# Gorilla-Lab-SCUT/GeoA3

Hardware: AMD Instinct MI355X
Metric: attack-iterations/sec (B=250, N=1024) (higher is better)
Workload: dtype f32; 1 GPU; configs[1]: PointNet 1024-pt, 250 instances sharded over 1 GPU(s) (250 on rank 0), full GeoA3 (CE + CD 1.0 + HD 0.1 + curvature 1.0 k=16), untargeted; instances_per_gpu=250, global_batch=250, npoint=1024, knn=16, classes=40, wide_mode=f16x2, presteps=150, parallelism=instance-sharded x1

## Files before the change

### geoa3_amd/csrc/pointnet_wide16.hip

```cpp
#include "pointnet_kernels.h"
#include "profile.h"

namespace {

constexpr int W16_THREADS = 256;
constexpr int W16_OCC = 2;
constexpr int W16_PTS = 128;
constexpr int W16_ROWS = W16_PTS + 2;
constexpr int W16_ROWB = 288;
constexpr int W16_PIECEB = W16_ROWS * W16_ROWB;
constexpr int W16_LDS = 2 * W16_PIECEB;

__global__ __launch_bounds__(W16_THREADS, W16_OCC) void wide16_kernel(WideArgs a, int slots_per_xcd) {
  constexpr int TAPS = 3;
  constexpr int GROUPS = 4;
  constexpr int KS = TAPS * 4;
  constexpr int PF = 2;
  extern __shared__ __attribute__((aligned(16))) unsigned char smem_raw[];
  __shared__ float s_max[4];
  __shared__ unsigned long long s_keys[4][GROUPS][32];
  const int tid = threadIdx.x, lane = tid & 63, wave = tid >> 6, p16 = lane & 15, q4 = lane >> 4, l31 = lane & 31,
            kh = lane >> 5;
  const int N = a.N, tiles = (N + W16_PTS - 1) / W16_PTS;
  constexpr int SPLIT = 8 / GROUPS;
  const int per_inst = tiles * SPLIT;
  const int xcd = blockIdx.x & 7, slot = blockIdx.x >> 3;
  const int inst_x = (a.B - xcd + 7) / 8;
  const int units = inst_x * per_inst;
  const half8* Wall = reinterpret_cast<const half8*>(a.Wh);
  if (tid == 0) s_max[0] = __int_as_float(__builtin_amdgcn_s_getreg((3 << 11) | 4) & 1);
  __syncthreads();
  bool late = __float_as_int(s_max[0]) != 0;
  const int nmine = units > slot ? (units - slot + slots_per_xcd - 1) / slots_per_xcd : 0;
  late = late && nmine > 0;
  int pend_b = -1, pend_co = 0, pend_n = 0;
  auto flush = [&]() {
    if (pend_b < 0) return;
    for (int i = kh; i < pend_n; i += 2)
      atomicMax(a.keys + (size_t)pend_b * a.Co + pend_co + i * 128 + l31, s_keys[wave][i][l31]);
    pend_b = -1;
  };
  for (int it = 0; it < nmine + (late ? 1 : 0); ++it) {
    const int u = slot + (it == nmine ? 0 : it) * slots_per_xcd;
    const int g_begin = late && it == nmine ? GROUPS / 2 : 0;
    const int g_end = late && it == 0 ? GROUPS / 2 : GROUPS;
    const int qi = u / per_inst, r = u - qi * per_inst;
    const int b = xcd + 8 * qi, tile = r / SPLIT, half = r - tile * SPLIT;
    const int n0 = tile * W16_PTS;
    const float* X = a.X + (size_t)b * a.sXb;
    float xv[2][4][8], xhalo = 0.f;
    {
      int ldx = a.ldX;
      asm volatile("" : "+s"(ldx));
#pragma unroll
      for (int pass = 0; pass < 2; ++pass) {
        const int n = n0 + pass * 64 + lane;
        const bool in = n < N;
        const float* px = X + (in ? n : 0);
#pragma unroll
        for (int oc = 0; oc < 4; ++oc)
#pragma unroll
          for (int i = 0; i < 8; ++i) {
            const float v = px[(size_t)(((wave + 4 * oc) * 8 + i) * ldx)];
            xv[pass][oc][i] = in ? v : 0.f;
          }
      }
      const int nh = tid < 128 ? n0 - 1 : n0 + W16_PTS;
      if (nh >= 0 && nh < N) xhalo = X[(size_t)((tid & 127) * ldx) + nh];
    }
    float m = __builtin_fabsf(xhalo);
#pragma unroll
    for (int pass = 0; pass < 2; ++pass)
#pragma unroll
      for (int oc = 0; oc < 4; ++oc)
#pragma unroll
        for (int i = 0; i < 8; ++i) m = fmaxf(m, __builtin_fabsf(xv[pass][oc][i]));
    m = wave_max(m);
    flush();
    __syncthreads();
    if (lane == 0) s_max[wave] = m;
    __syncthreads();
    m = fmaxf(fmaxf(s_max[0], s_max[1]), fmaxf(s_max[2], s_max[3]));
    unsigned E = (__float_as_uint(m) >> 23) & 0xffu;
    bool bad = E == 255u;
    E = sf_clamp(E);
    const float scale = sf_scale(E), unscale = a.unscale * sf_unscale(E);
#pragma unroll
    for (int pass = 0; pass < 2; ++pass) {
      const int p = 1 + pass * 64 + lane;
#pragma unroll
      for (int oc = 0; oc < 4; ++oc) {
        half8 hi, lo;
#pragma unroll
        for (int i = 0; i < 8; ++i) {
          const float xs = xv[pass][oc][i] * scale;
          bad |= xs != xs;
          _Float16 h, l;
          sf_split(xs, h, l);
          hi[i] = h;
          lo[i] = l;
        }
        unsigned char* dst = smem_raw + p * W16_ROWB + (wave + 4 * oc) * 16;
        *reinterpret_cast<half8*>(dst) = hi;
        *reinterpret_cast<half8*>(dst + W16_PIECEB) = lo;
      }
    }
    {
      const float xs = xhalo * scale;
      bad |= xs != xs;
      _Float16 h, l;
      sf_split(xs, h, l);
      unsigned char* dst = smem_raw + (tid < 128 ? 0 : W16_ROWS - 1) * W16_ROWB + (tid & 127) * 2;
      *reinterpret_cast<_Float16*>(dst) = h;
      *reinterpret_cast<_Float16*>(dst + W16_PIECEB) = l;
    }
    if (__syncthreads_or(bad))
      for (int c = tid; c < a.Co; c += W16_THREADS) atomicMax(a.keys + (size_t)b * a.Co + c, ~0ull);
    const unsigned char* abase = smem_raw + p16 * W16_ROWB + q4 * 16;
    auto a_rd = [&](int s, int t, half8& h, half8& l) {
      const unsigned char* ap = abase + ((s >> 2) + 16 * t) * W16_ROWB + (s & 3) * 64;
      h = *reinterpret_cast<const half8*>(ap);
      l = *reinterpret_cast<const half8*>(ap + W16_PIECEB);
    };
    auto wbase = [&](int g, int c2) {
      const int co = (half * GROUPS + g) * 128 + wave * 32 + 16 * c2;
      return Wall + (size_t)(co / 16) * KS * 2 * 64 + lane;
    };
    half8 wf[PF][2][2];
#pragma unroll
    for (int c2 = 0; c2 < 2; ++c2) {
      const half8* W0 = wbase(g_begin, c2);
#pragma unroll
      for (int f = 0; f < PF; ++f) {
        wf[f][c2][0] = W0[(size_t)(2 * f) * 64];
        wf[f][c2][1] = W0[(size_t)(2 * f + 1) * 64];
      }
    }
    half8 Ah[2][4], Al[2][4];
#pragma unroll
    for (int hf = 0; hf < 2; ++hf)
#pragma unroll
      for (int t = 0; t < 4; ++t) a_rd(0, 4 * hf + t, Ah[hf][t], Al[hf][t]);
#pragma unroll 1
    for (int g = g_begin; g < g_end; ++g) {
      const half8 *Wp[2], *Wn[2];
#pragma unroll
      for (int c2 = 0; c2 < 2; ++c2) {
        Wp[c2] = wbase(g, c2);
        Wn[c2] = wbase(g + 1 < g_end ? g + 1 : g, c2);
      }
      f32x4 acc[8][2];
#pragma unroll
      for (int t = 0; t < 8; ++t)
#pragma unroll
        for (int c2 = 0; c2 < 2; ++c2)
#pragma unroll
          for (int i = 0; i < 4; ++i) acc[t][c2][i] = 0.f;
#pragma unroll 1
      for (int s0 = 0; s0 < KS; s0 += PF) {
#pragma unroll
        for (int f = 0; f < PF; ++f) {
          const int s = s0 + f;
          const int sn = s + 1 < KS ? s + 1 : 0;
          half8 wh[2], wl[2];
#pragma unroll
          for (int c2 = 0; c2 < 2; ++c2) {
            wh[c2] = wf[f][c2][0];
            wl[c2] = wf[f][c2][1];
            const half8* src = s + PF < KS ? Wp[c2] + (size_t)(2 * 64) * (s + PF) : Wn[c2] + (size_t)(2 * 64) * (s + PF - KS);
            wf[f][c2][0] = src[0];
            wf[f][c2][1] = src[64];
          }
#pragma unroll
          for (int hf = 0; hf < 2; ++hf) {
            __builtin_amdgcn_sched_barrier(0);
#pragma unroll
            for (int t = 0; t < 4; ++t)
#pragma unroll
              for (int c2 = 0; c2 < 2; ++c2) {
                acc[4 * hf + t][c2] = __builtin_amdgcn_mfma_f32_16x16x32_f16(Ah[hf][t], wh[c2], acc[4 * hf + t][c2], 0, 0, 0);
                acc[4 * hf + t][c2] = __builtin_amdgcn_mfma_f32_16x16x32_f16(Ah[hf][t], wl[c2], acc[4 * hf + t][c2], 0, 0, 0);
                acc[4 * hf + t][c2] = __builtin_amdgcn_mfma_f32_16x16x32_f16(Al[hf][t], wh[c2], acc[4 * hf + t][c2], 0, 0, 0);
              }
            __builtin_amdgcn_sched_barrier(0);
#pragma unroll
            for (int t = 0; t < 4; ++t) a_rd(sn, 4 * hf + t, Ah[hf][t], Al[hf][t]);
          }
        }
      }
      const bool full = n0 + W16_PTS <= N;
#pragma unroll
      for (int c2 = 0; c2 < 2; ++c2) {
        float v = -__builtin_inff();
        int col = 0;
#pragma unroll
        for (int t = 0; t < 8; ++t)
#pragma unroll
          for (int r4 = 0; r4 < 4; ++r4) {
            const int n = n0 + 16 * t + 4 * q4 + r4;
            const bool gt = (full || n < N) && acc[t][c2][r4] > v;
            v = gt ? acc[t][c2][r4] : v;
            col = gt ? n : col;
          }
#pragma unroll
        for (int o = 16; o <= 32; o <<= 1) {
          const float ov = __shfl_xor(v, o, 64);
          const int oc = __shfl_xor(col, o, 64);
          const bool take = ov > v || (ov == v && oc < col);
          v = take ? ov : v;
          col = take ? oc : col;
        }
        if (lane < 16) s_keys[wave][g - g_begin][16 * c2 + lane] = wide_key(v * unscale, col);
      }
    }
    pend_b = b;
    pend_co = (half * GROUPS + g_begin) * 128 + wave * 32;
    pend_n = g_end - g_begin;
  }
  flush();
}

}

int launch_wide_max_split16(const WideArgs& a, hipStream_t s) {
  if (a.Co != 1024 || a.taps != 3 || !a.keys || !a.Wh) return GEOA3_ENOSUPPORT;
  geoa3_prof_begin(GEOA3_PROF_CONV5, s);
  if (!a.keys_clean &&
      hipMemsetAsync(a.keys, 0, (size_t)a.B * a.Co * sizeof(unsigned long long), s) != hipSuccess)
    return GEOA3_ELAUNCH;
  (void)hipFuncSetAttribute(reinterpret_cast<const void*>(wide16_kernel), hipFuncAttributeMaxDynamicSharedMemorySize, W16_LDS);
  constexpr int SLOTS = 32 * W16_OCC;
  hipLaunchKernelGGL(wide16_kernel, dim3(SLOTS * 8), dim3(W16_THREADS), W16_LDS, s, a, SLOTS);
  launch_wide_finalize(a, s);
  geoa3_prof_end(GEOA3_PROF_CONV5, s);
  GEOA3_CHECK_LAUNCH();
  return GEOA3_OK;
}
```

Measured before the change: 619.7 iterations/s of a 250-instance batch.

## Compute all output channels per tile in one unit, stash keys in LDS padding

Each work unit now covers all eight output-channel groups for a 128-point tile instead of splitting them into two halves. This removes the second staging of the same input tile (global loads, fp16 hi/lo split, LDS writes, barriers) per tile. Per-group max keys move from a separate static shared array into the unused padding bytes of the input rows, keeping the LDS footprint constant despite twice as many groups. Compile-time GEOA3_W16_CUT switches (default 0) add ablation paths that skip staging, the reduction, or weight prefetch; the trade-off is half as many units, which gives coarser load balance and a longer per-unit critical path.

```diff
diff --git a/geoa3_amd/csrc/pointnet_wide16.hip b/geoa3_amd/csrc/pointnet_wide16.hip
--- a/geoa3_amd/csrc/pointnet_wide16.hip
+++ b/geoa3_amd/csrc/pointnet_wide16.hip
@@ -11,19 +11,26 @@
 constexpr int W16_PIECEB = W16_ROWS * W16_ROWB;
 constexpr int W16_LDS = 2 * W16_PIECEB;
 
+#ifndef GEOA3_W16_CUT
+#define GEOA3_W16_CUT 0
+#endif
+
 __global__ __launch_bounds__(W16_THREADS, W16_OCC) void wide16_kernel(WideArgs a, int slots_per_xcd) {
   constexpr int TAPS = 3;
-  constexpr int GROUPS = 4;
+  constexpr int GROUPS = 8;
   constexpr int KS = TAPS * 4;
   constexpr int PF = 2;
   extern __shared__ __attribute__((aligned(16))) unsigned char smem_raw[];
   __shared__ float s_max[4];
-  __shared__ unsigned long long s_keys[4][GROUPS][32];
   const int tid = threadIdx.x, lane = tid & 63, wave = tid >> 6, p16 = lane & 15, q4 = lane >> 4, l31 = lane & 31,
             kh = lane >> 5;
+  auto key_slot = [&](int i, int l) {
+    const int k = (wave * GROUPS + i) * 32 + l;
+    unsigned char* row = smem_raw + (k >> 9) * W16_PIECEB + ((k >> 2) & 127) * W16_ROWB;
+    return reinterpret_cast<unsigned long long*>(row + 256 + (k & 3) * 8);
+  };
   const int N = a.N, tiles = (N + W16_PTS - 1) / W16_PTS;
-  constexpr int SPLIT = 8 / GROUPS;
-  const int per_inst = tiles * SPLIT;
+  const int per_inst = tiles;
   const int xcd = blockIdx.x & 7, slot = blockIdx.x >> 3;
   const int inst_x = (a.B - xcd + 7) / 8;
   const int units = inst_x * per_inst;
@@ -37,7 +44,7 @@
   auto flush = [&]() {
     if (pend_b < 0) return;
     for (int i = kh; i < pend_n; i += 2)
-      atomicMax(a.keys + (size_t)pend_b * a.Co + pend_co + i * 128 + l31, s_keys[wave][i][l31]);
+      atomicMax(a.keys + (size_t)pend_b * a.Co + pend_co + i * 128 + l31, *key_slot(i, l31));
     pend_b = -1;
   };
   for (int it = 0; it < nmine + (late ? 1 : 0); ++it) {
@@ -45,77 +52,84 @@
     const int g_begin = late && it == nmine ? GROUPS / 2 : 0;
     const int g_end = late && it == 0 ? GROUPS / 2 : GROUPS;
     const int qi = u / per_inst, r = u - qi * per_inst;
-    const int b = xcd + 8 * qi, tile = r / SPLIT, half = r - tile * SPLIT;
+    const int b = xcd + 8 * qi, tile = r;
     const int n0 = tile * W16_PTS;
     const float* X = a.X + (size_t)b * a.sXb;
-    float xv[2][4][8], xhalo = 0.f;
-    {
-      int ldx = a.ldX;
-      asm volatile("" : "+s"(ldx));
+    float unscale = a.unscale;
+    if (GEOA3_W16_CUT & 1) {
+      flush();
+      __syncthreads();
+    } else {
+      float xv[2][4][8], xhalo = 0.f;
+      {
+        int ldx = a.ldX;
+        asm volatile("" : "+s"(ldx));
+#pragma unroll
+        for (int pass = 0; pass < 2; ++pass) {
+          const int n = n0 + pass * 64 + lane;
+          const bool in = n < N;
+          const float* px = X + (in ? n : 0);
+#pragma unroll
+          for (int oc = 0; oc < 4; ++oc)
+#pragma unroll
+            for (int i = 0; i < 8; ++i) {
+              const float v = px[(size_t)(((wave + 4 * oc) * 8 + i) * ldx)];
+              xv[pass][oc][i] = in ? v : 0.f;
+            }
+        }
+        const int nh = tid < 128 ? n0 - 1 : n0 + W16_PTS;
+        if (nh >= 0 && nh < N) xhalo = X[(size_t)((tid & 127) * ldx) + nh];
+      }
+      float m = __builtin_fabsf(xhalo);
+#pragma unroll
+      for (int pass = 0; pass < 2; ++pass)
+#pragma unroll
+        for (int oc = 0; oc < 4; ++oc)
+#pragma unroll
+          for (int i = 0; i < 8; ++i) m = fmaxf(m, __builtin_fabsf(xv[pass][oc][i]));
+      m = wave_max(m);
+      flush();
+      __syncthreads();
+      if (lane == 0) s_max[wave] = m;
+      __syncthreads();
+      m = fmaxf(fmaxf(s_max[0], s_max[1]), fmaxf(s_max[2], s_max[3]));
+      unsigned E = (__float_as_uint(m) >> 23) & 0xffu;
+      bool bad = E == 255u;
+      E = sf_clamp(E);
+      const float scale = sf_scale(E);
+      unscale = a.unscale * sf_unscale(E);
 #pragma unroll
       for (int pass = 0; pass < 2; ++pass) {
-        const int n = n0 + pass * 64 + lane;
-        const bool in = n < N;
-        const float* px = X + (in ? n : 0);
-#pragma unroll
-        for (int oc = 0; oc < 4; ++oc)
+        const int p = 1 + pass * 64 + lane;
+#pragma unroll
+        for (int oc = 0; oc < 4; ++oc) {
+          half8 hi, lo;
 #pragma unroll
           for (int i = 0; i < 8; ++i) {
-            const float v = px[(size_t)(((wave + 4 * oc) * 8 + i) * ldx)];
-            xv[pass][oc][i] = in ? v : 0.f;
-          }
-      }
-      const int nh = tid < 128 ? n0 - 1 : n0 + W16_PTS;
-      if (nh >= 0 && nh < N) xhalo = X[(size_t)((tid & 127) * ldx) + nh];
+            const float xs = xv[pass][oc][i] * scale;
+            bad |= xs != xs;
+            _Float16 h, l;
+            sf_split(xs, h, l);
+            hi[i] = h;
+            lo[i] = l;
+          }
+          unsigned char* dst = smem_raw + p * W16_ROWB + (wave + 4 * oc) * 16;
+          *reinterpret_cast<half8*>(dst) = hi;
+          *reinterpret_cast<half8*>(dst + W16_PIECEB) = lo;
+        }
+      }
+      {
+        const float xs = xhalo * scale;
+        bad |= xs != xs;
+        _Float16 h, l;
+        sf_split(xs, h, l);
+        unsigned char* dst = smem_raw + (tid < 128 ? 0 : W16_ROWS - 1) * W16_ROWB + (tid & 127) * 2;
+        *reinterpret_cast<_Float16*>(dst) = h;
+        *reinterpret_cast<_Float16*>(dst + W16_PIECEB) = l;
+      }
+      if (__syncthreads_or(bad))
+        for (int c = tid; c < a.Co; c += W16_THREADS) atomicMax(a.keys + (size_t)b * a.Co + c, ~0ull);
     }
-    float m = __builtin_fabsf(xhalo);
-#pragma unroll
-    for (int pass = 0; pass < 2; ++pass)
-#pragma unroll
-      for (int oc = 0; oc < 4; ++oc)
-#pragma unroll
-        for (int i = 0; i < 8; ++i) m = fmaxf(m, __builtin_fabsf(xv[pass][oc][i]));
-    m = wave_max(m);
-    flush();
-    __syncthreads();
-    if (lane == 0) s_max[wave] = m;
-    __syncthreads();
-    m = fmaxf(fmaxf(s_max[0], s_max[1]), fmaxf(s_max[2], s_max[3]));
-    unsigned E = (__float_as_uint(m) >> 23) & 0xffu;
-    bool bad = E == 255u;
-    E = sf_clamp(E);
-    const float scale = sf_scale(E), unscale = a.unscale * sf_unscale(E);
-#pragma unroll
-    for (int pass = 0; pass < 2; ++pass) {
-      const int p = 1 + pass * 64 + lane;
-#pragma unroll
-      for (int oc = 0; oc < 4; ++oc) {
-        half8 hi, lo;
-#pragma unroll
-        for (int i = 0; i < 8; ++i) {
-          const float xs = xv[pass][oc][i] * scale;
-          bad |= xs != xs;
-          _Float16 h, l;
-          sf_split(xs, h, l);
-          hi[i] = h;
-          lo[i] = l;
-        }
-        unsigned char* dst = smem_raw + p * W16_ROWB + (wave + 4 * oc) * 16;
-        *reinterpret_cast<half8*>(dst) = hi;
-        *reinterpret_cast<half8*>(dst + W16_PIECEB) = lo;
-      }
-    }
-    {
-      const float xs = xhalo * scale;
-      bad |= xs != xs;
-      _Float16 h, l;
-      sf_split(xs, h, l);
-      unsigned char* dst = smem_raw + (tid < 128 ? 0 : W16_ROWS - 1) * W16_ROWB + (tid & 127) * 2;
-      *reinterpret_cast<_Float16*>(dst) = h;
-      *reinterpret_cast<_Float16*>(dst + W16_PIECEB) = l;
-    }
-    if (__syncthreads_or(bad))
-      for (int c = tid; c < a.Co; c += W16_THREADS) atomicMax(a.keys + (size_t)b * a.Co + c, ~0ull);
     const unsigned char* abase = smem_raw + p16 * W16_ROWB + q4 * 16;
     auto a_rd = [&](int s, int t, half8& h, half8& l) {
       const unsigned char* ap = abase + ((s >> 2) + 16 * t) * W16_ROWB + (s & 3) * 64;
@@ -123,7 +137,7 @@
       l = *reinterpret_cast<const half8*>(ap + W16_PIECEB);
     };
     auto wbase = [&](int g, int c2) {
-      const int co = (half * GROUPS + g) * 128 + wave * 32 + 16 * c2;
+      const int co = g * 128 + wave * 32 + 16 * c2;
       return Wall + (size_t)(co / 16) * KS * 2 * 64 + lane;
     };
     half8 wf[PF][2][2];
@@ -167,6 +181,7 @@
           for (int c2 = 0; c2 < 2; ++c2) {
             wh[c2] = wf[f][c2][0];
             wl[c2] = wf[f][c2][1];
+            if (GEOA3_W16_CUT & 4) continue;
             const half8* src = s + PF < KS ? Wp[c2] + (size_t)(2 * 64) * (s + PF) : Wn[c2] + (size_t)(2 * 64) * (s + PF - KS);
             wf[f][c2][0] = src[0];
             wf[f][c2][1] = src[64];
@@ -189,6 +204,13 @@
         }
       }
       const bool full = n0 + W16_PTS <= N;
+      if (GEOA3_W16_CUT & 2) {
+#pragma unroll
+        for (int t = 0; t < 8; ++t)
+#pragma unroll
+          for (int c2 = 0; c2 < 2; ++c2) asm volatile("" ::"v"(acc[t][c2]));
+        continue;
+      }
 #pragma unroll
       for (int c2 = 0; c2 < 2; ++c2) {
         float v = -__builtin_inff();
@@ -210,11 +232,12 @@
           v = take ? ov : v;
           col = take ? oc : col;
         }
-        if (lane < 16) s_keys[wave][g - g_begin][16 * c2 + lane] = wide_key(v * unscale, col);
+        if (lane < 16) *key_slot(g - g_begin, 16 * c2 + lane) = wide_key(v * unscale, col);
       }
     }
+    if (GEOA3_W16_CUT & 2) continue;
     pend_b = b;
-    pend_co = (half * GROUPS + g_begin) * 128 + wave * 32;
+    pend_co = g_begin * 128 + wave * 32;
     pend_n = g_end - g_begin;
   }
   flush();
```

New measurement: 630.9 iterations/s of a 250-instance batch (median of 6 runs). 1.02x the previous value.
